# beehive-lab/GPULlama3.java

Measured on AMD Instinct MI355X. Metric: tg128 tok/s (llama-bench), Llama-3-8B Q8_0, higher is better.
Workload: dtype i8; 1 GPU; Llama-3-8B-random Q8_0 random-weight GGUF-layout model, tg128 at depth 0 (one step = 128 decode tokens, logits D2H inside the timed region); parallelism=single GPU, ranks=1, ctx=648

## Files before the change

### gpullama3.java_amd/csrc/gl3_api.hip

```cpp
#include <chrono>
#include <cstdio>
#include <cstdlib>
#include <cstring>
#include <vector>

#include "gl3_ctx.h"
#include "gl3_batch_plan.h"
#include "gl3_decode_kernels.h"
#include "gl3_rowlane_kernels.h"
#include "gl3_veclane_kernels.h"
#include "gl3_moe_kernels.h"
#include "gl3_kv_copy.h"

using namespace gl3;

static std::string g_create_err;

static double now_ms() {
    return std::chrono::duration<double, std::milli>(std::chrono::steady_clock::now().time_since_epoch()).count();
}


static size_t matvec_smem(int pro, int epi, const Q8Mat& w) {
    const int nm = epi == EPI_SWIGLU ? 2 : 1;
// ... 21 lines not shown
}

template <int PRO, int EPI>
static hipError_t allow_big_lds() {
    hipError_t e = hipFuncSetAttribute((const void*)matvec_q8t_kernel<PRO, EPI, true>, hipFuncAttributeMaxDynamicSharedMemorySize, 160 * 1024 - 256);
    if (e != hipSuccess) return e;
    e = hipFuncSetAttribute((const void*)matvec_q8t_kernel<PRO, EPI, true, 4, false, true>, hipFuncAttributeMaxDynamicSharedMemorySize, 160 * 1024 - 256);
    if (e != hipSuccess) return e;
    e = hipFuncSetAttribute((const void*)matvec_q8t_kernel<PRO, EPI, true, 4, false, false, true>, hipFuncAttributeMaxDynamicSharedMemorySize, 160 * 1024 - 256);
    if (e != hipSuccess) return e;
    e = hipFuncSetAttribute((const void*)matvec_q8t_kernel<PRO, EPI, true, 4, false, true, true>, hipFuncAttributeMaxDynamicSharedMemorySize, 160 * 1024 - 256);
    if (e != hipSuccess) return e;
    return hipFuncSetAttribute((const void*)matvec_q8t_kernel<PRO, EPI, false>, hipFuncAttributeMaxDynamicSharedMemorySize, 160 * 1024 - 256);
}

static void launch_matvec(gl3_ctx* ctx, int pro, int epi, const Q8Mat& w, const Q8Mat* w2, const float* x,
                          const float* norm_w, float* out, const float* resid_in, float out_scale = 1.0f, const TpRec* tp = nullptr) {
    if (w.fmt != GL3_TYPE_Q8_0) {
        hipStream_t s = ctx->stream;
        static const bool vl_rms = env_flag("GL3_VL_RMS", true);
        static const bool ksplit_on = env_flag("GL3_VLQ", true);
        const bool ksplit_type = ksplit_on && w.vl && (w.fmt == GL3_FMT_Q8V || w.fmt == GL3_TYPE_Q4_0);
        const long vl_waves = (long)((w.rows + 7) / 8) * (epi == EPI_SWIGLU ? 2 : 1);
        const bool fuse_rms = pro == PRO_RMS && w.vl && vl_rms && vl_rms_fusable(w.k) && epi != EPI_RESID && !(ksplit_type && vl_waves <= 512);
        if (pro == PRO_RMS && !fuse_rms) {
            const size_t sm = (size_t)(w.k + 32) * 4 + ss_scratch_bytes(w.k) + 64;
            hipLaunchKernelGGL(rmsnorm_f32_kernel, dim3(1), dim3(256), sm, s, x, w.k, norm_w, ctx->d.rms_eps, ctx->xn);
            x = ctx->xn;
        }
        if (w.vl) {
            VlArgs v{};
            v.w = w.w; v.w2 = w2 ? w2->w : nullptr; v.rows = w.rows; v.k = w.k; v.x = x; v.out = out; v.resid_in = resid_in; v.out_scale = out_scale;
// ... 60 lines not shown
            else if (epi == EPI_RESID) hipLaunchKernelGGL((matvec_rl_kernel<WT_, EPI_RESID>), grid, dim3(RL_THREADS), sm, s, a); \
            else hipLaunchKernelGGL((matvec_rl_kernel<WT_, EPI_SWIGLU>), grid, dim3(RL_THREADS), sm, s, a); \
        } while (0)
        if (w.fmt == GL3_TYPE_F16) GL3_RL(WT_F16); else GL3_RL(WT_Q4_0);
#undef GL3_RL
        return;
    }
    static const bool nt = env_flag("GL3_NT", true);
    static const int max_wgs = getenv("GL3_WGS") ? atoi(getenv("GL3_WGS")) : 512;
    MatvecArgs a{};
    a.w = w.w; a.w2 = w2 ? w2->w : nullptr; a.rows = w.rows; a.k = w.k; a.ng = w.ng; a.nstrips = w.nstrips;
    a.x = x; a.norm_w = norm_w; a.eps = ctx->d.rms_eps; a.out = out; a.resid_in = resid_in; a.out_scale = out_scale;
    a.tp = tp;
    const int wgs = w.nstrips < max_wgs ? w.nstrips : max_wgs;
    const size_t smem = matvec_smem(pro, epi, w);
    if (pro == PRO_RMS && epi == EPI_STORE) launch_matvec_t<PRO_RMS, EPI_STORE>(ctx, a, wgs, smem, nt);
    else if (pro == PRO_QUANT && epi == EPI_RESID) {
        static const int wide_max = getenv("GL3_WIDE_STRIPS") ? atoi(getenv("GL3_WIDE_STRIPS")) : 256;
        const bool segs = w.ng > mv_seg_groups(8, EPI_RESID);
        if (w.nstrips <= wide_max && nt && tp && segs)
            launch_mv(ctx, matvec_q8t_kernel<PRO_QUANT, EPI_RESID, true, 8, false, true, true>, wgs, mv_threads(8), smem, a);
        else if (w.nstrips <= wide_max && nt && tp)
            launch_mv(ctx, matvec_q8t_kernel<PRO_QUANT, EPI_RESID, true, 8, false, true>, wgs, mv_threads(8), smem, a);
        else if (w.nstrips <= wide_max && nt && segs)
            launch_mv(ctx, matvec_q8t_kernel<PRO_QUANT, EPI_RESID, true, 8, false, false, true>, wgs, mv_threads(8), smem, a);
        else if (w.nstrips <= wide_max && nt)
            launch_mv(ctx, matvec_q8t_kernel<PRO_QUANT, EPI_RESID, true, 8>, wgs, mv_threads(8), smem, a);
        else launch_matvec_t<PRO_QUANT, EPI_RESID>(ctx, a, wgs, smem, nt);
    }
    else launch_matvec_t<PRO_RMS, EPI_SWIGLU>(ctx, a, wgs, smem, nt);
}
// ... 172 lines not shown

static int32_t all_gather(gl3_ctx* ctx, int which, int count_per_rank, Prof& pr) {
    if (!ctx->use_rccl) return GL3_OK;
    pr.begin(GL3_K_COLLECTIVE, 0);
    const int32_t r = gl3_all_gather(ctx, which, (size_t)count_per_rank);
    if (r != GL3_OK) return r;
    pr.end();
    return GL3_OK;
}

enum { ATT_LONG = 0, ATT_SHORT = 1, ATT_MID = 2 };
static int attn_mode(const gl3_ctx* ctx, int pos) {
    return (ctx->fused_attn_ok && pos < AF_MAXN) ? ATT_SHORT : pos < ctx->attn_mid ? ATT_MID : ATT_LONG;
}

static void launch_attention(gl3_ctx* ctx, int l, int which , int amode = ATT_LONG) {
    const gl3_model_desc& d = ctx->d;
    gl3_layer& L = ctx->layers[l];
    const size_t kv_layer = (size_t)d.ctx * ctx->kv_dim_l;
    const int kvmul = d.n_heads / d.n_kv_heads;
    AttnArgs aa{};
    aa.qkv = ctx->qkv; aa.kcache = ctx->kcache + l * kv_layer; aa.vcache = ctx->vcache + l * kv_layer;
    aa.rope_cr = ctx->rope_cr; aa.rope_ci = ctx->rope_ci; aa.qnorm = L.qnorm; aa.knorm = L.knorm; aa.bq = L.bq; aa.bk = L.bk; aa.bv = L.bv;
    aa.dyn = ctx->dyn_cur; aa.att = ctx->att; aa.xb = ctx->xb + (size_t)d.tp_rank * ctx->q_dim_l;
    aa.n_heads = ctx->heads_l; aa.n_kv_heads = ctx->kv_heads_l;
    aa.hs = d.head_size; aa.q_dim = ctx->q_dim_l; aa.kv_dim = ctx->kv_dim_l; aa.ctx = d.ctx;
    aa.eps = d.rms_eps; aa.arch = ctx->rope_arch; aa.att_mul = ctx->att_mul;
    const size_t sm1 = ((size_t)kvmul * d.head_size + (size_t)ATT_TT * (d.head_size + 4) + d.head_size) * 4;
    const int pv_rows = d.ctx < PV_ROWS ? d.ctx : PV_ROWS;
    aa.win = ctx->attn_win;
    aa.att_stride = (d.ctx + 3) & ~3;
    aa.att_t = ctx->att_t; aa.tmax = ctx->att_tmax; aa.sums = ctx->att_sums;
    aa.tp = tp_rec(ctx, l, TR_ATTN);
    const size_t sm2 = ((size_t)ctx->attn_win + (size_t)pv_rows * PV_COLS) * 4;
    if (which == 0 && amode == ATT_SHORT && ctx->fused_attn_ok) {
        attn_head_dispatch(d.head_size, [&](auto kern) { hipLaunchKernelGGL(kern, dim3(ctx->heads_l), dim3(256), attn_head_smem(d.head_size), ctx->stream, aa); });
        return;
    }
    static const bool scores_loop = env_flag("GL3_ATTN_SCORES_LOOP", true);
    if (which != 2 && amode == ATT_LONG && scores_loop && kvmul <= 4 && (d.head_size == 128 || d.head_size == 64)) {
        const dim3 sg(ctx->n_tsplit < SCL_WGS ? ctx->n_tsplit : SCL_WGS, ctx->kv_heads_l), sb(64 * (kvmul + SCL_LOADERS));
        const size_t sml = ((size_t)kvmul * d.head_size + 2 * (size_t)ATT_TT * (d.head_size + 4) + 2 * d.head_size) * 4;
        if (d.head_size == 128) hipLaunchKernelGGL(attn_scores_loop_kernel<128>, sg, sb, sml, ctx->stream, aa, ctx->n_tsplit);
        else hipLaunchKernelGGL(attn_scores_loop_kernel<64>, sg, sb, sml, ctx->stream, aa, ctx->n_tsplit);
    }
    else if (which != 2) hipLaunchKernelGGL(attn_scores_kernel, dim3(ctx->n_tsplit, ctx->kv_heads_l), dim3(64 * kvmul), sm1, ctx->stream, aa);
    if (which != 1 && amode == ATT_LONG) {
        const int exp_rows = (d.ctx + EXP_ROW - 1) / EXP_ROW;
        hipLaunchKernelGGL(attn_exp_kernel, dim3(exp_rows < EXP_GRID_MAX ? exp_rows : EXP_GRID_MAX, ctx->heads_l), dim3(256), 0, ctx->stream, aa, ctx->n_tsplit);
        hipLaunchKernelGGL(attn_sum_kernel, dim3(ctx->heads_l), dim3(256), attn_sum_smem(), ctx->stream, aa);
        hipLaunchKernelGGL(attn_pv_kernel, dim3(ctx->kv_heads_l * attn_pv_hq(kvmul) * (d.head_size / PV_COLS16)), dim3(64 * PV_WAVES), attn_pv_smem(), ctx->stream, aa);
// ... 16 lines not shown
    if (ctx->emb.fmt == GL3_TYPE_Q8_0)
        hipLaunchKernelGGL(embed_q8t_kernel, dim3(1), dim3(256), 0, s, ctx->emb.w, ctx->emb.ng, d.dim, ctx->dyn_cur, ctx->x, ctx->emb_scale,
                           (fmask & TF_EMBED) ? tp_rec(ctx, L_, 0) : (const TpRec*)nullptr,
                           fold ? reinterpret_cast<uint32_t*>(ctx->arena.base + GL3_ARENA_STEP) : (uint32_t*)nullptr);
    else if (ctx->emb.vl && ctx->emb.fmt == GL3_TYPE_F16) hipLaunchKernelGGL((embed_vl_kernel<WT_F16>), dim3(1), dim3(256), 0, s, ctx->emb.w, d.dim, ctx->dyn_cur, ctx->x, ctx->emb_scale, vl_step);
    else if (ctx->emb.vl && ctx->emb.fmt == GL3_FMT_Q8V) hipLaunchKernelGGL((embed_vl_kernel<WT_Q8_0>), dim3(1), dim3(256), 0, s, ctx->emb.w, d.dim, ctx->dyn_cur, ctx->x, ctx->emb_scale, vl_step);
    else if (ctx->emb.vl) hipLaunchKernelGGL((embed_vl_kernel<WT_Q4_0>), dim3(1), dim3(256), 0, s, ctx->emb.w, d.dim, ctx->dyn_cur, ctx->x, ctx->emb_scale, vl_step);
    else if (ctx->emb.fmt == GL3_TYPE_F16) hipLaunchKernelGGL((embed_rl_kernel<WT_F16>), dim3(1), dim3(256), 0, s, ctx->emb.w, d.dim, ctx->dyn_cur, ctx->x, ctx->emb_scale);
    else hipLaunchKernelGGL((embed_rl_kernel<WT_Q4_0>), dim3(1), dim3(256), 0, s, ctx->emb.w, d.dim, ctx->dyn_cur, ctx->x, ctx->emb_scale);
    pr.end();

    for (int l = 0; l < d.n_layers; ++l) {
        gl3_layer& L = ctx->layers[l];
        Gl3Range layer_range("layer", l);
        pr.begin(GL3_K_MATVEC_QKV, mv_bytes(L.wqkv) + d.dim * 4, q8);
        { Gl3Range g("rmsnorm + qkv"); launch_matvec(ctx, PRO_RMS, EPI_STORE, L.wqkv, nullptr, ctx->x, L.attn_norm, ctx->qkv, nullptr, 1.0f, (fmask & TF_QKV) && l > 0 ? tp_rec(ctx, l, TR_QKV) : nullptr); }
        pr.end();

        pr.begin(GL3_K_ATTENTION, 0);
        { Gl3Range g("rope + kv write + attention"); launch_attention(ctx, l, 0, amode); }
        pr.end();
        if (fold) fold_wait(ctx, l, TR_WAIT_XB, pr);
        else if ((r = all_gather(ctx, GB_XB, ctx->q_dim_l, pr)) != GL3_OK) return r;

        const size_t wo_off = ctx->wo_replicated ? 0 : (size_t)rank * ctx->dim_l;
        pr.begin(GL3_K_MATVEC_WO, mv_bytes(L.wo), q8);
        { Gl3Range g("wo + residual"); launch_matvec(ctx, PRO_QUANT, EPI_RESID, L.wo, nullptr, ctx->xb, nullptr, ctx->x + wo_off, ctx->x + wo_off, ctx->resid_scale,
                                                        (fmask & TF_WO) ? tp_rec(ctx, l, TR_WO) : nullptr); }
        pr.end();
        if (!ctx->wo_replicated && (r = all_gather(ctx, GB_X, ctx->dim_l, pr)) != GL3_OK) return r;

// ... 220 lines not shown
    } else {
        TRY(dmalloc(ctx, &ctx->x, d.dim));
        TRY(dmalloc(ctx, &ctx->xb, ctx->q_dim));
        TRY(dmalloc(ctx, &ctx->hb, d.hidden));
        TRY(dmalloc(ctx, &ctx->logits, d.vocab));
    }
    TRY(dmalloc(ctx, &ctx->att, (size_t)ctx->heads_l * ((d.ctx + 3) & ~3)));
    TRY(dmalloc(ctx, &ctx->att_t, attn_att_t_floats(ctx->kv_heads_l, d.n_heads / d.n_kv_heads, (d.ctx + 3) & ~3)));
    TRYHIP(hipMemset(ctx->att_t, 0, attn_att_t_floats(ctx->kv_heads_l, d.n_heads / d.n_kv_heads, (d.ctx + 3) & ~3) * 4));
    TRY(dmalloc(ctx, &ctx->att_tmax, (size_t)ctx->heads_l * ctx->n_tsplit));
    TRY(dmalloc(ctx, &ctx->att_sums, (size_t)ctx->heads_l));
    if (moe) TRY(moe_build_slots(ctx));
    TRYHIP((allow_big_lds<PRO_RMS, EPI_STORE>()));
    TRYHIP((allow_big_lds<PRO_QUANT, EPI_RESID>()));
    TRYHIP((allow_big_lds<PRO_RMS, EPI_SWIGLU>()));
    {
        ctx->fused_attn_ok = d.head_size % 4 == 0 && attn_head_smem(d.head_size) <= 150 * 1024 && !env_flag("GL3_NO_FUSED_ATTN", false);
        if (ctx->fused_attn_ok) {
            hipError_t ae = hipSuccess;
            attn_head_dispatch(d.head_size, [&](auto kern) { ae = hipFuncSetAttribute((const void*)kern, hipFuncAttributeMaxDynamicSharedMemorySize, 160 * 1024 - 256); });
            TRYHIP(ae);
        }
    }
    TRYHIP(hipFuncSetAttribute((const void*)matvec_q8t_kernel<PRO_QUANT, EPI_RESID, true, 8>, hipFuncAttributeMaxDynamicSharedMemorySize, 160 * 1024 - 256));
    TRYHIP(hipFuncSetAttribute((const void*)matvec_q8t_kernel<PRO_QUANT, EPI_RESID, true, 8, false, false, true>, hipFuncAttributeMaxDynamicSharedMemorySize, 160 * 1024 - 256));
    TRYHIP(hipFuncSetAttribute((const void*)matvec_q8t_kernel<PRO_QUANT, EPI_RESID, true, 8, false, true, true>, hipFuncAttributeMaxDynamicSharedMemorySize, 160 * 1024 - 256));
#define GL3_RL_LDS(...) TRYHIP(hipFuncSetAttribute((const void*)matvec_rl_kernel<__VA_ARGS__>, hipFuncAttributeMaxDynamicSharedMemorySize, 160 * 1024 - 256))
    GL3_RL_LDS(WT_F16, EPI_STORE); GL3_RL_LDS(WT_F16, EPI_RESID); GL3_RL_LDS(WT_F16, EPI_SWIGLU);
    GL3_RL_LDS(WT_Q4_0, EPI_STORE); GL3_RL_LDS(WT_Q4_0, EPI_RESID); GL3_RL_LDS(WT_Q4_0, EPI_SWIGLU);
#undef GL3_RL_LDS
    TRYHIP(hipFuncSetAttribute((const void*)rmsnorm_f32_kernel, hipFuncAttributeMaxDynamicSharedMemorySize, 160 * 1024 - 256));
    TRYHIP(hipFuncSetAttribute((const void*)attn_scores_kernel, hipFuncAttributeMaxDynamicSharedMemorySize, 128 * 1024));
    TRYHIP(hipFuncSetAttribute((const void*)attn_scores_loop_kernel<128>, hipFuncAttributeMaxDynamicSharedMemorySize, 128 * 1024));
    TRYHIP(hipFuncSetAttribute((const void*)attn_scores_loop_kernel<64>, hipFuncAttributeMaxDynamicSharedMemorySize, 128 * 1024));
    TRYHIP(hipFuncSetAttribute((const void*)attn_softmax_pv_kernel, hipFuncAttributeMaxDynamicSharedMemorySize, 150 * 1024));
// ... 1 lines not shown
    TRYHIP(hipFuncSetAttribute((const void*)attn_pv_kernel, hipFuncAttributeMaxDynamicSharedMemorySize, (int)attn_pv_smem()));
    {
        const char* wv = getenv("GL3_ATTN_WINDOW");
        int wmax = wv && *wv ? atoi(wv) : 16384;
        if (wmax < PV_ROWS || wmax % PV_ROWS != 0 || wmax > 16384) return bail(GL3_E_ARG, "GL3_ATTN_WINDOW must be a multiple of 1024 between 1024 and 16384");
        ctx->attn_win = d.ctx <= wmax ? ((d.ctx + 3) & ~3) : wmax;
        const char* mv = getenv("GL3_ATTN_MID");
        ctx->attn_mid = mv && *mv ? atoi(mv) : 768;
    }
    TRY(dmalloc(ctx, &ctx->dyn, GL3_DYN_INTS));
    ctx->dyn_cur = ctx->dyn;
    TRY(dmalloc(ctx, &ctx->argmax, 2 + 2 * AMX_WGS));
    TRYHIP(hipMemset(ctx->argmax, 0, (2 + 2 * AMX_WGS) * sizeof(int)));
    if (d.flags & GL3_FLAG_LAYER_TAPS) TRY(dmalloc(ctx, &ctx->taps, (size_t)d.n_layers * d.dim));
    TRYHIP(hipHostMalloc((void**)&ctx->h_dyn, GL3_DYN_INTS * sizeof(int)));
    TRYHIP(hipHostMalloc((void**)&ctx->h_logits, (size_t)d.vocab * 4));
    TRYHIP(hipHostMalloc((void**)&ctx->h_argmax, sizeof(int)));
    {
        const bool int8_path = d.weight_type == GL3_TYPE_Q8_0 && !(d.flags & GL3_FLAG_F32_ACTIVATION);
        const bool vl_path = !int8_path && !(d.flags & GL3_FLAG_SCALAR_DOT);
        if (d.max_batch > 1 && (int8_path || vl_path)) TRY(gl3_prefill_alloc(ctx));
    }
    if (getenv("GL3_DEBUG_ALLOC")) {
        fprintf(stderr, "[gl3 alloc] ctx %p emb %p (+%zu) kcache %p vcache %p (%zu floats) x %p qkv %p xb %p hb %p logits %p att %p xn %p\n", (void*)ctx, (void*)ctx->emb.w,
                ctx->emb.bytes(), (void*)ctx->kcache, (void*)ctx->vcache, kvn, (void*)ctx->x, (void*)ctx->qkv, (void*)ctx->xb, (void*)ctx->hb, (void*)ctx->logits, (void*)ctx->att, (void*)ctx->xn);
        for (size_t l = 0; l < ctx->layers.size(); ++l) {
            const gl3_layer& L = ctx->layers[l];
            fprintf(stderr, "[gl3 alloc]   layer %zu wqkv %p (+%zu) wo %p (+%zu) w1 %p (+%zu) w3 %p w2 %p (+%zu)\n", l, (void*)L.wqkv.w, L.wqkv.bytes(), (void*)L.wo.w, L.wo.bytes(),
                    (void*)L.w1.w, L.w1.bytes(), (void*)L.w3.w, (void*)L.w2.w, L.w2.bytes());
        }
// ... 561 lines not shown

int32_t gl3_profile_kernel(gl3_ctx* ctx, int32_t klass, int32_t iters, double* out_us, uint64_t* bytes_per_launch) {
    if (!ctx || !out_us || iters <= 0) return GL3_E_ARG;
    if (!ctx->finalized) GL3_FAIL(GL3_E_STATE, "profile before gl3_finalize");
    if (klass < GL3_K_MATVEC_QKV || klass > GL3_K_OTHER) GL3_FAIL(GL3_E_ARG, "kernel class cannot be profiled");
    GL3_HIP(hipSetDevice(ctx->d.device));
    const gl3_model_desc& d = ctx->d;
    const int rank = d.tp_rank;
    hipEvent_t e0, e1;
    GL3_HIP(hipEventCreate(&e0)); GL3_HIP(hipEventCreate(&e1));
    auto sweep = [&]() {
        const int nl = klass == GL3_K_MATVEC_LOGITS ? 1 : d.n_layers;
        for (int l = 0; l < nl; ++l) {
            gl3_layer& L = ctx->layers[l];
            switch (klass) {
            case GL3_K_MATVEC_QKV: launch_matvec(ctx, PRO_RMS, EPI_STORE, L.wqkv, nullptr, ctx->x, L.attn_norm, ctx->qkv, nullptr); break;
            case GL3_K_MATVEC_WO: launch_matvec(ctx, PRO_QUANT, EPI_RESID, L.wo, nullptr, ctx->xb, nullptr, ctx->qkv, nullptr); break;
            case GL3_K_MATVEC_GATEUP: launch_matvec(ctx, PRO_RMS, EPI_SWIGLU, L.w1, &L.w3, ctx->x, L.ffn_norm, ctx->hb + (size_t)rank * ctx->hidden_l, nullptr); break;
            case GL3_K_MATVEC_DOWN: launch_matvec(ctx, PRO_QUANT, EPI_RESID, L.w2, nullptr, ctx->hb, nullptr, ctx->qkv, nullptr); break;
            case GL3_K_ATTENTION: launch_attention(ctx, l, 0, attn_mode(ctx, ctx->h_dyn[1])); break;
            case GL3_K_OTHER: launch_attention(ctx, l, 2, attn_mode(ctx, ctx->h_dyn[1]) == ATT_LONG ? ATT_LONG : ATT_MID); break;
            default: launch_matvec(ctx, PRO_RMS, EPI_STORE, ctx->wcls, nullptr, ctx->x, ctx->out_norm, ctx->logits + (size_t)rank * ctx->vocab_l, nullptr); break;
            }
        }
        return nl;
    };
    struct Quiet { gl3_ctx* c; ~Quiet() { c->tp_quiet = false; } } quiet{ctx};
    ctx->tp_quiet = true;
    sweep();
    GL3_HIP(hipEventRecord(e0, ctx->stream));
    long n = 0;
// ... 272 lines not shown
```

### gpullama3.java_amd/csrc/gl3_decode_kernels.h

```cpp
#pragma once
#include <hip/hip_runtime.h>
#include <stdint.h>

#include "gl3_seqsum.h"

namespace gl3 {

constexpr int TILE_BYTES = 2176;
constexpr int MV_AUX = 4;
__host__ __device__ constexpr int mv_threads(int npw) { return 64 * (npw + MV_AUX); }

enum { PRO_RMS = 0, PRO_QUANT = 1 };
enum { EPI_STORE = 0, EPI_RESID = 1, EPI_SWIGLU = 2 };
__host__ __device__ constexpr int mv_ch(int epi) { return epi == EPI_SWIGLU ? 4 : 8; }
__host__ __device__ constexpr int mv_seg_groups(int npw, int epi) { return npw * mv_ch(epi); }

typedef float v4f __attribute__((ext_vector_type(4)));

#ifdef GL3_MV_TIMING
__device__ long long gl3_mv_stamp[32];
#define ATT_STAMP(i) do { if (blockIdx.x == 0 && threadIdx.x == 0) gl3_mv_stamp[i] = wall_clock64(); } while (0)
#define MV_STAMP(i, cond) do { if (blockIdx.x == 0 && (cond)) gl3_mv_stamp[i] = clock64(); } while (0)
#define PV_T(...) __VA_ARGS__
constexpr int MV_WG_STAMPS = 1024;
__device__ unsigned long long gl3_mv_wg_stamp[MV_WG_STAMPS][8];
#define MV_WG_TIME(v) v = (unsigned long long)wall_clock64()
#define MV_WG_PUT(s, v, cond) do { if (blockIdx.x < MV_WG_STAMPS && blockIdx.y == 0 && (cond)) atomicMax(&gl3_mv_wg_stamp[blockIdx.x][s], v); } while (0)
#else
// ... 54 lines not shown
struct MatvecArgs {
    const uint8_t* w;
    const uint8_t* w2;
    int rows;
    int k;
    int ng;
    int nstrips;
    const float* x;
    const float* norm_w;
    float eps;
    float* out;
    const float* resid_in;
    float out_scale;
    const struct MoeSlots* moe;
    const TpRec* tp;
};

struct MoeSlots {
    const int* sel;
    size_t sel_stride;
    int x_slot_stride, out_slot_stride;
    int n_sel, sh_rows;
    const uint8_t* sh_w;
    const uint8_t* sh_w2;
    float* sh_out;
};

__device__ __forceinline__ void lds_barrier() { asm volatile("s_waitcnt lgkmcnt(0)\n\ts_barrier" ::: "memory"); }

struct LdsBarrier { __device__ __forceinline__ void operator()() const { lds_barrier(); } };
// ... 227 lines not shown

    __builtin_amdgcn_s_setprio(3);
    const int ta = t - 64 * MV_PRODUCERS;
    const int nquads = a.k >> 2;
    float scale = 1.0f;
    constexpr int NXV = (PRO == PRO_RMS) ? 5 : 14;
    float4 nwv[5], xv[NXV];
    if (!TPF) {
#pragma unroll
        for (int i = 0; i < NXV; ++i) xv[i] = *reinterpret_cast<const float4*>(a.x + 4 * min(ta + 256 * i, nquads - 1));
    }
    if (PRO == PRO_RMS) {
#pragma unroll
        for (int i = 0; i < 5; ++i) nwv[i] = *reinterpret_cast<const float4*>(a.norm_w + 4 * min(ta + 256 * i, nquads - 1));
    }
    __syncthreads();
    if (TPF) {
        if (a.tp->w.flags) tp_wait(a.tp->w);
#pragma unroll
        for (int i = 0; i < NXV; ++i) xv[i] = *reinterpret_cast<const float4*>(a.x + 4 * min(ta + 256 * i, nquads - 1));
    }
    SubBarrier aux_sync{&sync_w[0], MV_AUX, 0};
    if (PRO == PRO_RMS) {
        if (nquads <= NXV * 256) {
#pragma unroll
            for (int i = 0; i < NXV; ++i) { const int qd = ta + 256 * i; if (qd < nquads) *reinterpret_cast<float4*>(xf + 4 * qd) = xv[i]; }
        } else {
            for (int qd = ta; qd < nquads; qd += 256)
                *reinterpret_cast<float4*>(xf + 4 * qd) = *reinterpret_cast<const float4*>(a.x + 4 * qd);
        }
        if (ta < 32) xf[a.k + ta] = 0.f;
// ... 36 lines not shown
        }
    } else {
        for (int qd = ta; qd < nquads; qd += 256) {
            float4 v = *reinterpret_cast<const float4*>(a.x + 4 * qd);
            if (PRO == PRO_RMS) {
                const float4 w = *reinterpret_cast<const float4*>(a.norm_w + 4 * qd);
                v.x = w.x * (scale * v.x); v.y = w.y * (scale * v.y); v.z = w.z * (scale * v.z); v.w = w.w * (scale * v.w);
            }
            quantize_quad(v, qd, xq, xs);
        }
    }
    aux_sync();
    if (ta == 0) __hip_atomic_store(&sync_w[1], 1, __ATOMIC_RELEASE, __HIP_MEMORY_SCOPE_WORKGROUP);
    if (wave != MV_PRODUCERS) return;

    int it = 0;
    for (int strip = blockIdx.x; strip < a.nstrips; strip += gridDim.x, ++it) {
        const float* pb = pbuf + (size_t)(it & 1) * NM * a.ng * 64;
        v4f acc[NM];
#pragma unroll
        for (int m = 0; m < NM; ++m) acc[m] = (v4f){0.f, 0.f, 0.f, 0.f};
        for (int b = 0; b < nbatch; ++b) {
            if (SEGS) lds_barrier(); else __syncthreads();
            MV_STAMP(16 + 2 * it, lane == 0 && it < 4 && b == nbatch - 1);
            MV_WG_TIME(wg_t1);
            int g = b * SEG;
            const int ge = SEGS ? min(g + SEG, a.ng) : a.ng;
            for (; g + 8 <= ge; g += 8) {
                float av[NM][8];
#pragma unroll
                for (int m = 0; m < NM; ++m)
#pragma unroll
                    for (int u = 0; u < 8; ++u) av[m][u] = pb[(size_t)m * a.ng * 64 + (g + u) * 64 + lane];
#pragma unroll
                for (int u = 0; u < 8; ++u)
#pragma unroll
// ... 1 lines not shown
            }
            for (; g < ge; ++g)
#pragma unroll
                for (int m = 0; m < NM; ++m)
                    acc[m] = __builtin_amdgcn_mfma_f32_16x16x4f32(pb[(size_t)m * a.ng * 64 + g * 64 + lane], 1.0f, acc[m], 0, 0, 0);
        }
        MV_STAMP(17 + 2 * it, lane == 0 && it < 4);
        MV_WG_TIME(wg_t2);
        if ((lane & 15) < 4) {
            const int r = lane & 3;
            const int row = strip * 16 + 4 * (lane >> 4) + r;
            if (row < a.rows) {
                const float v0 = r == 0 ? acc[0][0] : r == 1 ? acc[0][1] : r == 2 ? acc[0][2] : acc[0][3];
                float res;
                if (EPI == EPI_STORE) res = v0 * a.out_scale;
                if (EPI == EPI_RESID) res = a.resid_in ? a.resid_in[row] + v0 * a.out_scale : v0 * a.out_scale;
                if (EPI == EPI_SWIGLU) {
                    const float v1 = r == 0 ? acc[NM - 1][0] : r == 1 ? acc[NM - 1][1] : r == 2 ? acc[NM - 1][2] : acc[NM - 1][3];
                    const float gte = v0 / (float)(1.0 + exp(-(double)v0));
                    res = gte * v1;
                }
                a.out[row] = res;
                if (TPF) tp_push_store(a.tp->p, a.out + row, res);
            }
        }
        PV_T(asm volatile("s_waitcnt vmcnt(0)" ::: "memory");)
        MV_WG_TIME(wg_t0);
        MV_WG_PUT(2, wg_t1, lane == 0); MV_WG_PUT(3, wg_t2, lane == 0); MV_WG_PUT(4, wg_t0, lane == 0);
    }
    if (TPF && a.tp->p.npeers) tp_publish(a.tp->p, gridDim.x);
}

static __global__ __launch_bounds__(256) void embed_q8t_kernel(const uint8_t* __restrict__ emb, int ng, int dim,
                                                         const int* __restrict__ dyn, float* __restrict__ x, float emb_scale,
                                                         const TpRec* tp = nullptr, uint32_t* step = nullptr) {
    if (step) {
        const uint32_t s = *step;
        __syncthreads();
// ... 293 lines not shown
        if (t0 + r < t1) {
            my_score = a.att_mul != 0.f ? score * a.att_mul : score / sqrt_hs;
            a.att[(size_t)(kvh * kvmul + hq) * a.att_stride + t0 + r] = my_score;
        }
        const float m = wave_max(my_score);
        if (r == 0) a.tmax[(size_t)(kvh * kvmul + hq) * n_tiles_max + sp] = m;
    }
    PV_T(if (blockIdx.x == 0 && blockIdx.y == 0 && t == 0) { gl3_mv_stamp[5] = cbw_; gl3_mv_stamp[6] = clock64() - cts_; gl3_mv_stamp[7] = cnt; })
}

constexpr int AF_MAXN = 128;
__host__ __device__ inline size_t attn_head_smem(int hs, int group = 1) {
    return ((size_t)group * hs + (size_t)AF_MAXN * (hs + 4) + (size_t)AF_MAXN * hs + (size_t)group * AF_MAXN + hs + 16) * 4;
}

template <int HS>
static __global__ __launch_bounds__(256, 1) void attn_head_kernel(const AttnArgs a) {
    extern __shared__ __attribute__((aligned(16))) float sm[];
    const int hs = HS > 0 ? HS : a.hs, kvmul = a.n_heads / a.n_kv_heads, half = hs >> 1, pitch = hs + 4, q4 = hs >> 2;
    const int q4sh = (q4 & (q4 - 1)) == 0 ? __ffs(q4) - 1 : -1;
    auto row_of = [&](int i) { return q4sh >= 0 ? i >> q4sh : i / q4; };
    auto col_of = [&](int i, int row) { return q4sh >= 0 ? i & (q4 - 1) : i - row * q4; };
    const int G = a.group > 1 ? a.group : 1;
    float* q_s = sm;
    float* kt = q_s + G * hs;
    float* vt = kt + AF_MAXN * pitch;
    float* e_s = vt + AF_MAXN * hs;
    float* cr_s = e_s + G * AF_MAXN;
    float* ci_s = cr_s + half;
    float* red = ci_s + half;
    const int t = threadIdx.x, lane = t & 63, wave = t >> 6;
    const int h0 = blockIdx.x * G, kvh = h0 / kvmul;
    const bool owner = (h0 % kvmul) == 0;
    const int bt = blockIdx.y;
    const int pos = a.seqv ? a.posv[bt] : a.dyn[1], n = pos + 1;
    const size_t kvoff = a.seqv ? (size_t)a.seqv[bt] * a.seq_stride : 0;
    const float* qkv = a.qkv + (size_t)bt * a.qkv_stride;
    float* kcache = a.kcache + kvoff;
    float* vcache = a.vcache + kvoff;
    ATT_STAMP(0);
    const int nk4 = pos * q4;
    constexpr int KMAX = 16;
    float4 kreg[KMAX], vreg[KMAX];
    const bool in_regs = nk4 <= KMAX * 256;
    const int per = in_regs ? (nk4 + 255) >> 8 : 0;
#pragma unroll
    for (int u = 0; u < KMAX; ++u) {
        kreg[u] = make_float4(0.f, 0.f, 0.f, 0.f);
        vreg[u] = make_float4(0.f, 0.f, 0.f, 0.f);
        if (u < per) {
            const int i = min(t + u * 256, nk4 - 1), ri = row_of(i);
            const size_t off = (size_t)ri * a.kv_dim + kvh * hs + 4 * col_of(i, ri);
            kreg[u] = *reinterpret_cast<const float4*>(kcache + off);
            vreg[u] = *reinterpret_cast<const float4*>(vcache + off);
        }
    }
    for (int i = t; i < G * hs; i += 256) q_s[i] = a.bq ? qkv[h0 * hs + i] + a.bq[h0 * hs + i] : qkv[h0 * hs + i];
    for (int i = t; i < half; i += 256) { cr_s[i] = a.rope_cr[(size_t)pos * half + i]; ci_s[i] = a.rope_ci[(size_t)pos * half + i]; }
    float* krow = kt + pos * pitch;
    for (int i = t; i < hs; i += 256) {
        krow[i] = a.bk ? qkv[a.q_dim + kvh * hs + i] + a.bk[kvh * hs + i] : qkv[a.q_dim + kvh * hs + i];
        vt[pos * hs + i] = a.bv ? qkv[a.q_dim + a.kv_dim + kvh * hs + i] + a.bv[kvh * hs + i] : qkv[a.q_dim + a.kv_dim + kvh * hs + i];
    }
    if (in_regs) {
#pragma unroll
        for (int u = 0; u < KMAX; ++u) {
            const int i = t + u * 256;
            if (i < nk4) {
                const int ri = row_of(i), ci = col_of(i, ri);
                *reinterpret_cast<float4*>(kt + ri * pitch + 4 * ci) = kreg[u];
                *reinterpret_cast<float4*>(vt + ri * hs + 4 * ci) = vreg[u];
            }
        }
    } else {
        for (int i = t; i < nk4; i += 256) {
            const int ri = row_of(i), ci = col_of(i, ri);
            const size_t off = (size_t)ri * a.kv_dim + kvh * hs + 4 * ci;
            *reinterpret_cast<float4*>(kt + ri * pitch + 4 * ci) = *reinterpret_cast<const float4*>(kcache + off);
            *reinterpret_cast<float4*>(vt + ri * hs + 4 * ci) = *reinterpret_cast<const float4*>(vcache + off);
        }
    }
    __syncthreads();
    ATT_STAMP(1);
    if (a.arch == 1) {
        for (int vec = wave; vec <= G; vec += 4)
            head_rmsnorm_wave(vec < G ? q_s + vec * hs : krow, vec < G ? a.qnorm : a.knorm, hs, a.eps, lane);
        __syncthreads();
    }
    for (int g = 0; g < G; ++g) rope_head(q_s + g * hs, hs, cr_s, ci_s, a.arch, t, 256);
    rope_head(krow, hs, cr_s, ci_s, a.arch, t, 256);
    __syncthreads();
    if (owner) {
        for (int i = t; i < hs; i += 256) {
            kcache[(size_t)pos * a.kv_dim + kvh * hs + i] = krow[i];
            vcache[(size_t)pos * a.kv_dim + kvh * hs + i] = vt[pos * hs + i];
        }
    }
    ATT_STAMP(2);
    const float sqrt_hs = (float)sqrt((double)hs);
    float sc = -INFINITY;
    for (int idx = t; idx < G * n; idx += 256) {
        const int g = idx / n, tt = idx - g * n;
        const float* q = q_s + g * hs;
        const float* kk = kt + tt * pitch;
        float score = 0.f;
        float4 qv = *reinterpret_cast<const float4*>(q), kv = *reinterpret_cast<const float4*>(kk);
        for (int j = 4; j < hs; j += 4) {
            const float4 qn = *reinterpret_cast<const float4*>(q + j), kn = *reinterpret_cast<const float4*>(kk + j);
            score = score + qv.x * kv.x; score = score + qv.y * kv.y; score = score + qv.z * kv.z; score = score + qv.w * kv.w;
            qv = qn; kv = kn;
// ... 82 lines not shown
            const int q3 = __builtin_amdgcn_update_dpp(0, q0, 0xFF, 0xf, 0xf, false);
            const int el = (h0 + g) * hs + j;
            if ((lane & 3) == 0)
                *reinterpret_cast<uint32_t*>(a.xq_out + bdq_offset(el >> 2, bt, a.xq_slots)) = (uint32_t)q0 | ((uint32_t)q1 << 8) | ((uint32_t)q2 << 16) | ((uint32_t)q3 << 24);
            if ((lane & 31) == 0) a.xs_out[bds_offset(el >> 5, bt, a.xq_slots)] = (float)(_Float16)qs;
        } else {
            float* o = a.xb + (size_t)bt * a.xb_stride + (size_t)(h0 + g) * hs + j;
            *o = acc;
            if (a.tp) tp_push_store(a.tp->p, o, acc);
        }
    }
    ATT_STAMP(6);
    if (a.tp) tp_publish(a.tp->p, gridDim.x * gridDim.y * 4);
}

template <typename F>
static inline void attn_head_dispatch(int hs, F&& f) {
    if (hs == 128) f(attn_head_kernel<128>);
    else if (hs == 64) f(attn_head_kernel<64>);
    else f(attn_head_kernel<0>);
}

constexpr int PV_COLS = 16;
constexpr int PV_ROWS = 1024;

static __global__ __launch_bounds__(256) void attn_softmax_pv_kernel(const AttnArgs a) {
    extern __shared__ __attribute__((aligned(16))) float e_s[];
    const int hs = a.hs, kvmul = a.n_heads / a.n_kv_heads;
    const int nj = hs / PV_COLS;
    const int h = blockIdx.x / nj, j0 = (blockIdx.x % nj) * PV_COLS;
    const int t = threadIdx.x, lane = t & 63, wave = t >> 6, kvh = h / kvmul;
    const int n = a.dyn[1] + 1;
    float* vbuf = e_s + a.win;
    const float* vbase = a.vcache + kvh * hs + j0;
    constexpr int SU = PV_ROWS * 4 / 256;
// ... 376 lines not shown
```

Before: 476.4 tok/s.

## Fuse RoPE and KV-cache write into QKV matvec epilogue for short attention

Adds an EPI_QKV epilogue to the Q8 matvec that applies rotary embedding to Q and K rows and writes K/V straight into the layer's KV cache. The fused attention kernel gets a PRE variant that skips the q/k load-with-bias, rope, rmsnorm and cache-write phases, reading K/V including the current position from the cache. This removes a synchronized serial rope/cache stage inside each attention block at the cost of rope-table loads in the matvec epilogue. It is enabled only for single-GPU, non-biased, non-qk-norm, rope_arch 0 models in the short-attention mode.

```diff
diff --git a/gpullama3.java_amd/csrc/gl3_api.hip b/gpullama3.java_amd/csrc/gl3_api.hip
--- a/gpullama3.java_amd/csrc/gl3_api.hip
+++ b/gpullama3.java_amd/csrc/gl3_api.hip
@@ -59,8 +59,11 @@
     return hipFuncSetAttribute((const void*)matvec_q8t_kernel<PRO, EPI, false>, hipFuncAttributeMaxDynamicSharedMemorySize, 160 * 1024 - 256);
 }
 
+struct QkvRopeDst { float* k; float* v; int pos_stride; };
+
 static void launch_matvec(gl3_ctx* ctx, int pro, int epi, const Q8Mat& w, const Q8Mat* w2, const float* x,
-                          const float* norm_w, float* out, const float* resid_in, float out_scale = 1.0f, const TpRec* tp = nullptr) {
+                          const float* norm_w, float* out, const float* resid_in, float out_scale = 1.0f, const TpRec* tp = nullptr,
+                          const QkvRopeDst* qr = nullptr) {
     if (w.fmt != GL3_TYPE_Q8_0) {
         hipStream_t s = ctx->stream;
         static const bool vl_rms = env_flag("GL3_VL_RMS", true);
@@ -151,7 +154,15 @@
     a.tp = tp;
     const int wgs = w.nstrips < max_wgs ? w.nstrips : max_wgs;
     const size_t smem = matvec_smem(pro, epi, w);
-    if (pro == PRO_RMS && epi == EPI_STORE) launch_matvec_t<PRO_RMS, EPI_STORE>(ctx, a, wgs, smem, nt);
+    if (qr) {
+        a.kdst = qr->k; a.vdst = qr->v; a.kv_pos_stride = qr->pos_stride;
+        a.rope_cr = ctx->rope_cr; a.rope_ci = ctx->rope_ci; a.dyn = ctx->dyn_cur;
+        a.q_dim = ctx->q_dim_l; a.kv_dim = ctx->kv_dim_l; a.hs = ctx->d.head_size;
+        if (nt && a.ng > mv_seg_groups(4, EPI_QKV)) launch_mv(ctx, matvec_q8t_kernel<PRO_RMS, EPI_QKV, true, 4, false, false, true>, wgs, mv_threads(4), smem, a);
+        else if (nt) launch_mv(ctx, matvec_q8t_kernel<PRO_RMS, EPI_QKV, true>, wgs, mv_threads(4), smem, a);
+        else launch_mv(ctx, matvec_q8t_kernel<PRO_RMS, EPI_QKV, false>, wgs, mv_threads(4), smem, a);
+    }
+    else if (pro == PRO_RMS && epi == EPI_STORE) launch_matvec_t<PRO_RMS, EPI_STORE>(ctx, a, wgs, smem, nt);
     else if (pro == PRO_QUANT && epi == EPI_RESID) {
         static const int wide_max = getenv("GL3_WIDE_STRIPS") ? atoi(getenv("GL3_WIDE_STRIPS")) : 256;
         const bool segs = w.ng > mv_seg_groups(8, EPI_RESID);
@@ -354,6 +365,16 @@
     return (ctx->fused_attn_ok && pos < AF_MAXN) ? ATT_SHORT : pos < ctx->attn_mid ? ATT_MID : ATT_LONG;
 }
 
+static bool qkv_rope_layer(const gl3_ctx* ctx, int l, int amode) {
+    static const bool on = env_flag("GL3_QKV_ROPE", true);
+    const gl3_model_desc& d = ctx->d;
+    const gl3_layer& L = ctx->layers[l];
+    if (!on || amode != ATT_SHORT || !ctx->fused_attn_ok) return false;
+    if (d.tp_size != 1 || (d.flags & GL3_FLAG_FORCE_RCCL) || ctx->use_rccl || ctx->tp_fold) return false;
+    if (L.wqkv.fmt != GL3_TYPE_Q8_0 || ctx->rope_arch != 0 || d.head_size % 16 != 0) return false;
+    return !(L.bq || L.bk || L.bv || L.qnorm || L.knorm);
+}
+
 static void launch_attention(gl3_ctx* ctx, int l, int which , int amode = ATT_LONG) {
     const gl3_model_desc& d = ctx->d;
     gl3_layer& L = ctx->layers[l];
@@ -374,7 +395,9 @@
     aa.tp = tp_rec(ctx, l, TR_ATTN);
     const size_t sm2 = ((size_t)ctx->attn_win + (size_t)pv_rows * PV_COLS) * 4;
     if (which == 0 && amode == ATT_SHORT && ctx->fused_attn_ok) {
-        attn_head_dispatch(d.head_size, [&](auto kern) { hipLaunchKernelGGL(kern, dim3(ctx->heads_l), dim3(256), attn_head_smem(d.head_size), ctx->stream, aa); });
+        auto go = [&](auto kern) { hipLaunchKernelGGL(kern, dim3(ctx->heads_l), dim3(256), attn_head_smem(d.head_size), ctx->stream, aa); };
+        if (qkv_rope_layer(ctx, l, amode)) attn_head_dispatch<true>(d.head_size, go);
+        else attn_head_dispatch(d.head_size, go);
         return;
     }
     static const bool scores_loop = env_flag("GL3_ATTN_SCORES_LOOP", true);
@@ -421,7 +444,11 @@
         gl3_layer& L = ctx->layers[l];
         Gl3Range layer_range("layer", l);
         pr.begin(GL3_K_MATVEC_QKV, mv_bytes(L.wqkv) + d.dim * 4, q8);
-        { Gl3Range g("rmsnorm + qkv"); launch_matvec(ctx, PRO_RMS, EPI_STORE, L.wqkv, nullptr, ctx->x, L.attn_norm, ctx->qkv, nullptr, 1.0f, (fmask & TF_QKV) && l > 0 ? tp_rec(ctx, l, TR_QKV) : nullptr); }
+        { Gl3Range g("rmsnorm + qkv");
+          const size_t kv_layer = (size_t)d.ctx * ctx->kv_dim_l;
+          const QkvRopeDst qr{ctx->kcache + l * kv_layer, ctx->vcache + l * kv_layer, ctx->kv_dim_l};
+          launch_matvec(ctx, PRO_RMS, EPI_STORE, L.wqkv, nullptr, ctx->x, L.attn_norm, ctx->qkv, nullptr, 1.0f, (fmask & TF_QKV) && l > 0 ? tp_rec(ctx, l, TR_QKV) : nullptr,
+                        qkv_rope_layer(ctx, l, amode) ? &qr : nullptr); }
         pr.end();
 
         pr.begin(GL3_K_ATTENTION, 0);
@@ -672,11 +699,15 @@
     TRYHIP((allow_big_lds<PRO_RMS, EPI_STORE>()));
     TRYHIP((allow_big_lds<PRO_QUANT, EPI_RESID>()));
     TRYHIP((allow_big_lds<PRO_RMS, EPI_SWIGLU>()));
+    TRYHIP(hipFuncSetAttribute((const void*)matvec_q8t_kernel<PRO_RMS, EPI_QKV, true>, hipFuncAttributeMaxDynamicSharedMemorySize, 160 * 1024 - 256));
+    TRYHIP(hipFuncSetAttribute((const void*)matvec_q8t_kernel<PRO_RMS, EPI_QKV, true, 4, false, false, true>, hipFuncAttributeMaxDynamicSharedMemorySize, 160 * 1024 - 256));
+    TRYHIP(hipFuncSetAttribute((const void*)matvec_q8t_kernel<PRO_RMS, EPI_QKV, false>, hipFuncAttributeMaxDynamicSharedMemorySize, 160 * 1024 - 256));
     {
         ctx->fused_attn_ok = d.head_size % 4 == 0 && attn_head_smem(d.head_size) <= 150 * 1024 && !env_flag("GL3_NO_FUSED_ATTN", false);
         if (ctx->fused_attn_ok) {
             hipError_t ae = hipSuccess;
-            attn_head_dispatch(d.head_size, [&](auto kern) { ae = hipFuncSetAttribute((const void*)kern, hipFuncAttributeMaxDynamicSharedMemorySize, 160 * 1024 - 256); });
+            auto big = [&](auto kern) { if (ae == hipSuccess) ae = hipFuncSetAttribute((const void*)kern, hipFuncAttributeMaxDynamicSharedMemorySize, 160 * 1024 - 256); };
+            attn_head_dispatch(d.head_size, big); attn_head_dispatch<true>(d.head_size, big);
             TRYHIP(ae);
         }
     }
@@ -708,6 +739,8 @@
     TRYHIP(hipMemset(ctx->argmax, 0, (2 + 2 * AMX_WGS) * sizeof(int)));
     if (d.flags & GL3_FLAG_LAYER_TAPS) TRY(dmalloc(ctx, &ctx->taps, (size_t)d.n_layers * d.dim));
     TRYHIP(hipHostMalloc((void**)&ctx->h_dyn, GL3_DYN_INTS * sizeof(int)));
+    memset(ctx->h_dyn, 0, GL3_DYN_INTS * sizeof(int));
+    TRYHIP(hipMemset(ctx->dyn, 0, GL3_DYN_INTS * sizeof(int)));
     TRYHIP(hipHostMalloc((void**)&ctx->h_logits, (size_t)d.vocab * 4));
     TRYHIP(hipHostMalloc((void**)&ctx->h_argmax, sizeof(int)));
     {
@@ -1299,7 +1332,12 @@
         for (int l = 0; l < nl; ++l) {
             gl3_layer& L = ctx->layers[l];
             switch (klass) {
-            case GL3_K_MATVEC_QKV: launch_matvec(ctx, PRO_RMS, EPI_STORE, L.wqkv, nullptr, ctx->x, L.attn_norm, ctx->qkv, nullptr); break;
+            case GL3_K_MATVEC_QKV: {
+                const QkvRopeDst qr{ctx->qkv + ctx->q_dim_l, ctx->qkv + ctx->q_dim_l + ctx->kv_dim_l, 0};
+                launch_matvec(ctx, PRO_RMS, EPI_STORE, L.wqkv, nullptr, ctx->x, L.attn_norm, ctx->qkv, nullptr, 1.0f, nullptr,
+                              qkv_rope_layer(ctx, l, attn_mode(ctx, ctx->h_dyn[1])) ? &qr : nullptr);
+                break;
+            }
             case GL3_K_MATVEC_WO: launch_matvec(ctx, PRO_QUANT, EPI_RESID, L.wo, nullptr, ctx->xb, nullptr, ctx->qkv, nullptr); break;
             case GL3_K_MATVEC_GATEUP: launch_matvec(ctx, PRO_RMS, EPI_SWIGLU, L.w1, &L.w3, ctx->x, L.ffn_norm, ctx->hb + (size_t)rank * ctx->hidden_l, nullptr); break;
             case GL3_K_MATVEC_DOWN: launch_matvec(ctx, PRO_QUANT, EPI_RESID, L.w2, nullptr, ctx->hb, nullptr, ctx->qkv, nullptr); break;
diff --git a/gpullama3.java_amd/csrc/gl3_decode_kernels.h b/gpullama3.java_amd/csrc/gl3_decode_kernels.h
--- a/gpullama3.java_amd/csrc/gl3_decode_kernels.h
+++ b/gpullama3.java_amd/csrc/gl3_decode_kernels.h
@@ -11,7 +11,7 @@
 __host__ __device__ constexpr int mv_threads(int npw) { return 64 * (npw + MV_AUX); }
 
 enum { PRO_RMS = 0, PRO_QUANT = 1 };
-enum { EPI_STORE = 0, EPI_RESID = 1, EPI_SWIGLU = 2 };
+enum { EPI_STORE = 0, EPI_RESID = 1, EPI_SWIGLU = 2, EPI_QKV = 3 };
 __host__ __device__ constexpr int mv_ch(int epi) { return epi == EPI_SWIGLU ? 4 : 8; }
 __host__ __device__ constexpr int mv_seg_groups(int npw, int epi) { return npw * mv_ch(epi); }
 
@@ -96,6 +96,12 @@
     float out_scale;
     const struct MoeSlots* moe;
     const TpRec* tp;
+    float* kdst;
+    float* vdst;
+    const float* rope_cr;
+    const float* rope_ci;
+    const int* dyn;
+    int q_dim, kv_dim, hs, kv_pos_stride;
 };
 
 struct MoeSlots {
@@ -353,7 +359,14 @@
 #pragma unroll
         for (int i = 0; i < 5; ++i) nwv[i] = *reinterpret_cast<const float4*>(a.norm_w + 4 * min(ta + 256 * i, nquads - 1));
     }
+    float rcr = 0.f, rci = 0.f;
     __syncthreads();
+    int qpos = 0;
+    if (EPI == EPI_QKV) {
+        int qidx = 1;
+        asm volatile("" : "+v"(qidx));
+        qpos = a.dyn[qidx];
+    }
     if (TPF) {
         if (a.tp->w.flags) tp_wait(a.tp->w);
 #pragma unroll
@@ -420,12 +433,18 @@
     if (ta == 0) __hip_atomic_store(&sync_w[1], 1, __ATOMIC_RELEASE, __HIP_MEMORY_SCOPE_WORKGROUP);
     if (wave != MV_PRODUCERS) return;
 
+    auto rope_ld = [&](int strip) {
+        const int row = min(strip * 16 + 4 * (lane >> 4) + (lane & 3), a.rows - 1);
+        const size_t ri = (size_t)qpos * (a.hs >> 1) + ((row % a.hs) >> 1);
+        rcr = a.rope_cr[ri]; rci = a.rope_ci[ri];
+    };
     int it = 0;
     for (int strip = blockIdx.x; strip < a.nstrips; strip += gridDim.x, ++it) {
         const float* pb = pbuf + (size_t)(it & 1) * NM * a.ng * 64;
         v4f acc[NM];
 #pragma unroll
         for (int m = 0; m < NM; ++m) acc[m] = (v4f){0.f, 0.f, 0.f, 0.f};
+        if (EPI == EPI_QKV) rope_ld(strip);
         for (int b = 0; b < nbatch; ++b) {
             if (SEGS) lds_barrier(); else __syncthreads();
             MV_STAMP(16 + 2 * it, lane == 0 && it < 4 && b == nbatch - 1);
@@ -457,14 +476,24 @@
                 const float v0 = r == 0 ? acc[0][0] : r == 1 ? acc[0][1] : r == 2 ? acc[0][2] : acc[0][3];
                 float res;
                 if (EPI == EPI_STORE) res = v0 * a.out_scale;
+                if (EPI == EPI_QKV) {
+                    const float ve = (r < 2 ? acc[0][0] : acc[0][2]) * a.out_scale, vo = (r < 2 ? acc[0][1] : acc[0][3]) * a.out_scale;
+                    const float rot = (r & 1) ? mul_f32_scalar(ve, rci) + mul_f32_scalar(vo, rcr) : mul_f32_scalar(ve, rcr) - mul_f32_scalar(vo, rci);
+                    const size_t kvrow = (size_t)qpos * a.kv_pos_stride;
+                    if (row < a.q_dim) a.out[row] = rot;
+                    else if (row < a.q_dim + a.kv_dim) a.kdst[kvrow + (row - a.q_dim)] = rot;
+                    else a.vdst[kvrow + (row - a.q_dim - a.kv_dim)] = v0 * a.out_scale;
+                }
                 if (EPI == EPI_RESID) res = a.resid_in ? a.resid_in[row] + v0 * a.out_scale : v0 * a.out_scale;
                 if (EPI == EPI_SWIGLU) {
                     const float v1 = r == 0 ? acc[NM - 1][0] : r == 1 ? acc[NM - 1][1] : r == 2 ? acc[NM - 1][2] : acc[NM - 1][3];
                     const float gte = v0 / (float)(1.0 + exp(-(double)v0));
                     res = gte * v1;
                 }
-                a.out[row] = res;
-                if (TPF) tp_push_store(a.tp->p, a.out + row, res);
+                if (EPI != EPI_QKV) {
+                    a.out[row] = res;
+                    if (TPF) tp_push_store(a.tp->p, a.out + row, res);
+                }
             }
         }
         PV_T(asm volatile("s_waitcnt vmcnt(0)" ::: "memory");)
@@ -788,7 +817,7 @@
     return ((size_t)group * hs + (size_t)AF_MAXN * (hs + 4) + (size_t)AF_MAXN * hs + (size_t)group * AF_MAXN + hs + 16) * 4;
 }
 
-template <int HS>
+template <int HS, bool PRE = false>
 static __global__ __launch_bounds__(256, 1) void attn_head_kernel(const AttnArgs a) {
     extern __shared__ __attribute__((aligned(16))) float sm[];
     const int hs = HS > 0 ? HS : a.hs, kvmul = a.n_heads / a.n_kv_heads, half = hs >> 1, pitch = hs + 4, q4 = hs >> 2;
@@ -813,11 +842,13 @@
     float* kcache = a.kcache + kvoff;
     float* vcache = a.vcache + kvoff;
     ATT_STAMP(0);
-    const int nk4 = pos * q4;
+    const int nk4 = (PRE ? n : pos) * q4;
     constexpr int KMAX = 16;
     float4 kreg[KMAX], vreg[KMAX];
     const bool in_regs = nk4 <= KMAX * 256;
     const int per = in_regs ? (nk4 + 255) >> 8 : 0;
+    float qreg = 0.f;
+    if (PRE) qreg = qkv[h0 * hs + min(t, G * hs - 1)];
 #pragma unroll
     for (int u = 0; u < KMAX; ++u) {
         kreg[u] = make_float4(0.f, 0.f, 0.f, 0.f);
@@ -829,12 +860,17 @@
             vreg[u] = *reinterpret_cast<const float4*>(vcache + off);
         }
     }
-    for (int i = t; i < G * hs; i += 256) q_s[i] = a.bq ? qkv[h0 * hs + i] + a.bq[h0 * hs + i] : qkv[h0 * hs + i];
-    for (int i = t; i < half; i += 256) { cr_s[i] = a.rope_cr[(size_t)pos * half + i]; ci_s[i] = a.rope_ci[(size_t)pos * half + i]; }
     float* krow = kt + pos * pitch;
-    for (int i = t; i < hs; i += 256) {
-        krow[i] = a.bk ? qkv[a.q_dim + kvh * hs + i] + a.bk[kvh * hs + i] : qkv[a.q_dim + kvh * hs + i];
-        vt[pos * hs + i] = a.bv ? qkv[a.q_dim + a.kv_dim + kvh * hs + i] + a.bv[kvh * hs + i] : qkv[a.q_dim + a.kv_dim + kvh * hs + i];
+    if (PRE) {
+        if (t < G * hs) q_s[t] = qreg;
+        for (int i = t + 256; i < G * hs; i += 256) q_s[i] = qkv[h0 * hs + i];
+    } else {
+        for (int i = t; i < G * hs; i += 256) q_s[i] = a.bq ? qkv[h0 * hs + i] + a.bq[h0 * hs + i] : qkv[h0 * hs + i];
+        for (int i = t; i < half; i += 256) { cr_s[i] = a.rope_cr[(size_t)pos * half + i]; ci_s[i] = a.rope_ci[(size_t)pos * half + i]; }
+        for (int i = t; i < hs; i += 256) {
+            krow[i] = a.bk ? qkv[a.q_dim + kvh * hs + i] + a.bk[kvh * hs + i] : qkv[a.q_dim + kvh * hs + i];
+            vt[pos * hs + i] = a.bv ? qkv[a.q_dim + a.kv_dim + kvh * hs + i] + a.bv[kvh * hs + i] : qkv[a.q_dim + a.kv_dim + kvh * hs + i];
+        }
     }
     if (in_regs) {
 #pragma unroll
@@ -856,18 +892,20 @@
     }
     __syncthreads();
     ATT_STAMP(1);
-    if (a.arch == 1) {
-        for (int vec = wave; vec <= G; vec += 4)
-            head_rmsnorm_wave(vec < G ? q_s + vec * hs : krow, vec < G ? a.qnorm : a.knorm, hs, a.eps, lane);
+    if (!PRE) {
+        if (a.arch == 1) {
+            for (int vec = wave; vec <= G; vec += 4)
+                head_rmsnorm_wave(vec < G ? q_s + vec * hs : krow, vec < G ? a.qnorm : a.knorm, hs, a.eps, lane);
+            __syncthreads();
+        }
+        for (int g = 0; g < G; ++g) rope_head(q_s + g * hs, hs, cr_s, ci_s, a.arch, t, 256);
+        rope_head(krow, hs, cr_s, ci_s, a.arch, t, 256);
         __syncthreads();
-    }
-    for (int g = 0; g < G; ++g) rope_head(q_s + g * hs, hs, cr_s, ci_s, a.arch, t, 256);
-    rope_head(krow, hs, cr_s, ci_s, a.arch, t, 256);
-    __syncthreads();
-    if (owner) {
-        for (int i = t; i < hs; i += 256) {
-            kcache[(size_t)pos * a.kv_dim + kvh * hs + i] = krow[i];
-            vcache[(size_t)pos * a.kv_dim + kvh * hs + i] = vt[pos * hs + i];
+        if (owner) {
+            for (int i = t; i < hs; i += 256) {
+                kcache[(size_t)pos * a.kv_dim + kvh * hs + i] = krow[i];
+                vcache[(size_t)pos * a.kv_dim + kvh * hs + i] = vt[pos * hs + i];
+            }
         }
     }
     ATT_STAMP(2);
@@ -980,11 +1018,11 @@
     if (a.tp) tp_publish(a.tp->p, gridDim.x * gridDim.y * 4);
 }
 
-template <typename F>
+template <bool PRE = false, typename F>
 static inline void attn_head_dispatch(int hs, F&& f) {
-    if (hs == 128) f(attn_head_kernel<128>);
-    else if (hs == 64) f(attn_head_kernel<64>);
-    else f(attn_head_kernel<0>);
+    if (hs == 128) f(attn_head_kernel<128, PRE>);
+    else if (hs == 64) f(attn_head_kernel<64, PRE>);
+    else f(attn_head_kernel<0, PRE>);
 }
 
 constexpr int PV_COLS = 16;
```

Result: no change. 478.1 tok/s (median of 6 runs) (+0.3%).
